# humanoid-path-planner/hpp-fcl

Measured on AMD Instinct MI355X. Metric: narrow-phase queries/s (collision+distance), higher is better.
Workload: dtype f32; 1 GPU; cfg3_convex32_distance_nesterov; request=distance, gather=none

## Files before the change

### hpp-fcl_amd/csrc/hfcl_dev.hpp

```cpp
#pragma once
#include <hip/hip_runtime.h>

#include <cstdint>
#include <cstring>
#include <type_traits>

#include "../../include/hppfcl_amd.h"
#include "hfcl_bvh.hpp"
#include "hfcl_bvh_shape.hpp"
#include "hfcl_pair.hpp"

using namespace hfcl;

#ifndef HFCL_WPE_GJK_W2
#define HFCL_WPE_GJK_W2 2
#endif
#ifndef HFCL_WPE_GJK
#define HFCL_WPE_GJK 3
#endif
#ifndef HFCL_WPE_GJK64
#define HFCL_WPE_GJK64 2
#endif
#ifndef HFCL_WPE_PRIM
#define HFCL_WPE_PRIM 2
#endif
#ifndef HFCL_WPE_EPA32
#define HFCL_WPE_EPA32 2
#endif
#ifndef HFCL_WPE_EPA64
#define HFCL_WPE_EPA64 1
#endif
#ifndef HFCL_WPE_BVH
#define HFCL_WPE_BVH 1
#endif

enum { B_CLOSED = 0, B_PRIM = 1, B_CC = 2, B_PC = 3, B_CP = 4, B_BVH = 5, B_UNSUPPORTED = 6, B_LARGE = 7, B_BVHSHAPE = 8, B_TRI = 9, B_COUNT = 10 };
constexpr int B_CURVED0 = B_COUNT + 4;
constexpr int CTR_SHAPE_TICKET = 2 * B_COUNT + 4, CTR_SHAPE_DEFER = 2 * B_COUNT + 5;
constexpr int CTR_DIST_SUSP = 2 * B_COUNT + 6;
constexpr int CTR_SHAPE_DIST_SUSP = 2 * B_COUNT + 7;
constexpr int CTR_DIST_TICKET = 2 * B_COUNT + 8;
constexpr int CTR_SHAPE_DIST_TICKET = 2 * B_COUNT + 9;
constexpr int CTR_EPA_CC_OVER = 2 * B_COUNT + 10;
constexpr int CTR_SHAPE_FINISH_OVER = 2 * B_COUNT + 11;
constexpr int CTR_SHAPE_DEFER_MARK = 2 * B_COUNT + 13;
constexpr int CTR_DIST_RERUN = 2 * B_COUNT + 14, CTR_SHAPE_DIST_RERUN = 2 * B_COUNT + 15;
constexpr int N_COUNTERS = 2 * B_COUNT + 16;

constexpr int K_CONVEX_LARGE = 21;

__host__ __device__ inline int bucket_of(int k1, int k2, bool distance_mode = false) {
  if (distance_mode && (k1 == K_TRIANGLE || k2 == K_TRIANGLE)) return B_UNSUPPORTED;
  const bool large = (k1 == K_CONVEX_LARGE) || (k2 == K_CONVEX_LARGE);
  if (k1 == K_CONVEX_LARGE) k1 = K_CONVEX;
  if (k2 == K_CONVEX_LARGE) k2 = K_CONVEX;
  if ((k1 == K_BVH) != (k2 == K_BVH)) {
    const int o = (k1 == K_BVH) ? k2 : k1;
    return (kind_is_prim(o) || o == K_CONVEX || kind_is_flat(o)) ? B_BVHSHAPE : B_UNSUPPORTED;
  }
  if ((k1 == K_TRIANGLE || k2 == K_TRIANGLE) && !kind_is_flat(k1) && !kind_is_flat(k2)) {
    const int o = (k1 == K_TRIANGLE) ? k2 : k1;
    return (o == K_TRIANGLE || kind_is_prim(o) || o == K_CONVEX) ? B_TRI : B_UNSUPPORTED;
  }
  const int c = pair_class(k1, k2);
  if (large && c == CLS_CONVEX) return B_LARGE;
  if (c == CLS_CLOSED) return B_CLOSED;
  if (c == CLS_PRIM_GJK) return B_PRIM;
  if (c == CLS_BVH) return B_BVH;
  if (c == CLS_CONVEX) {
    if (k1 == K_CONVEX && k2 == K_CONVEX) return B_CC;
    return (k1 == K_CONVEX) ? B_CP : B_PC;
  }
  return B_UNSUPPORTED;
}

template <typename T>
struct NbrEntry;
template <> struct alignas(16) NbrEntry<float> { float x, y, z; uint32_t id; };
template <> struct alignas(32) NbrEntry<double> { double x, y, z; uint32_t id; uint32_t pad_; };

// ... 657 lines not shown
```

### hpp-fcl_amd/csrc/hfcl_host.hip

```cpp
#include "hfcl_host.hpp"
#include "hfcl_plan.hpp"

static thread_local std::string g_last_error;
void set_error(const std::string& s) { g_last_error = s; }
void hfcl_internal_set_error(const char* msg) { g_last_error = msg ? msg : ""; }

static void free_retired_graphs(hfcl_lib* lib);

static uint32_t total_count(const hfcl_lib* lib, int i) {
  if (lib->last_host) return one_count(lib->acc_counts, i);
  uint32_t c = lib->h_counts ? one_count(lib->h_counts, i) : 0u;
  if (lib->last_split && lib->helper && lib->helper->h_counts) c += one_count(lib->helper->h_counts, i);
  return c;
}

static int ensure_device(int device) {
  int n = 0;
  hipError_t e = hipGetDeviceCount(&n);
  if (e != hipSuccess || n == 0) {
    set_error("no HIP device available (hipGetDeviceCount): the engine has no CPU fallback");
    return HFCL_ERR_NO_DEVICE;
  }
  if (device < 0 || device >= n) {
    set_error("device index out of range");
// ... 149 lines not shown
  }
  lib->h_kinds = kinds;
  std::vector<float> v32(3 * n_vertices + 3);
  for (size_t i = 0; i < 3 * n_vertices; ++i) v32[i] = float(vertices[i]);
  hfcl_lib::Tables& t = lib->own;
  reset_all(t.shapes64, t.shapes32, t.kinds, t.verts64, t.verts32);
  bool ok = true;
  ok = ok && t.shapes64.grow(n_shapes) == hipSuccess;
  ok = ok && t.shapes32.grow(n_shapes) == hipSuccess;
  ok = ok && t.kinds.grow(n_shapes) == hipSuccess;
  ok = ok && t.verts64.grow(3 * n_vertices + 3) == hipSuccess;
  ok = ok && t.verts32.grow(3 * n_vertices + 3) == hipSuccess;
  if (ok) {
    ok = ok && hipMemcpy(t.shapes64, s64.data(), n_shapes * sizeof(DShape<double>), hipMemcpyHostToDevice) == hipSuccess;
    ok = ok && hipMemcpy(t.shapes32, s32.data(), n_shapes * sizeof(DShape<float>), hipMemcpyHostToDevice) == hipSuccess;
    ok = ok && hipMemcpy(t.kinds, kinds.data(), n_shapes, hipMemcpyHostToDevice) == hipSuccess;
    if (n_vertices) {
      ok = ok && hipMemcpy(t.verts64, vertices, 3 * n_vertices * sizeof(double), hipMemcpyHostToDevice) == hipSuccess;
      ok = ok && hipMemcpy(t.verts32, v32.data(), 3 * n_vertices * sizeof(float), hipMemcpyHostToDevice) == hipSuccess;
    }
  }
  share_tables(lib, lib);
  return ok;
}

static const char* const* option_keys() {
  static const char* const keys[] = {
      "closed_staged", "split", "epa_cc_staged", "epa_records_aside", "epa_general_staged", "shape_finish_tiers", "shape_finish_aside",
      "epa_general_staged_min", "epa64_two_streams", "epa_cc_staged_min", "pipe_chunk", "bvh_filter", "bvh_shape_lane", "shape_coop",
      "bvh_cut_ticks", "shape_cut_ticks", "bvh_coop", "bvhd_budget", "bvhd_pool", "shape_dist_pool", "pool_rerun", "bvh_walk_early_coop",
      "bvh_walk_rounds", "bvh_walk_order", "mesh_beside", "mesh_prio", "shape_walk", "shape_walk_sort", "shape_walk_budget", "shape_walk_min", "gjk_beside_max", "epa_direct_max", "bvh_walk_k", "bvh_walk_budget", "shape_dist_leaf_min", "shape_dist_starve", "bvhd_leaf_min", "bvhd_starve",
      "bvhd_part_min", "shape_dist_budget", "bvh_budget0_coop", "shape_budget0", "shape_budget", "shape_leaf_cost", "shape_levels",
      "climb_min", "bvh_budget", "bvh_budget0", "bvh_levels", "cvx_w", "epa_resume_slots", "bvh_task_slots", "bvh_force_wide",
      "pipe_trace", "scene_chunk", "scene_cull_chunk", "scene_pairs_small_max", nullptr};
  return keys;
}
static int parse_list(const char* v, uint32_t* out, int first, int cap, uint32_t lo, uint32_t hi) {
  int k = first;
  for (const char* p = v; *p && k < cap; ++k) {
    const long long x = atoll(p);
    out[k] = uint32_t(std::min<long long>(std::max<long long>(x, lo), hi));
    while (*p && *p != ',') ++p;
    if (*p == ',') ++p;
  }
  return k - first;
}
static int apply_option(hfcl_lib* lib, const std::string& key, const char* v) {
  const long long i = atoll(v);
  const bool on = i != 0;
  auto u32 = [&](long long lo) { return uint32_t(std::min<long long>(std::max(i, lo), 0xFFFFFFFFll)); };
  if (key == "closed_staged") lib->opt.closed_staged = on;
  else if (key == "split") lib->opt.split = i >= 2 ? 2 : (i == 1 ? 1 : 0);
  else if (key == "epa_cc_staged") lib->opt.epa_cc_staged = on;
  else if (key == "epa_records_aside") lib->opt.records_aside = on;
  else if (key == "epa_general_staged") {
    if (on && !HFCL_KEEP_AB_FORMS) return HFCL_ERR_INVALID_ARGUMENT;
    lib->opt.epa_general_staged = on;
  }
  else if (key == "shape_finish_tiers") lib->opt.shape_finish_tiers = on;
  else if (key == "shape_finish_aside") lib->opt.shape_finish_aside = on;
  else if (key == "epa_general_staged_min") lib->opt.epa_general_staged_min = size_t(std::max(0ll, i));
  else if (key == "epa64_two_streams") lib->opt.epa64_two_streams = on;
  else if (key == "epa_cc_staged_min") lib->opt.epa_cc_staged_min = size_t(std::max(0ll, i));
  else if (key == "pipe_chunk") lib->opt.pipe_chunk = strtoull(v, nullptr, 10);
  else if (key == "bvh_filter") {
    if (on && !HFCL_KEEP_AB_FORMS) return HFCL_ERR_INVALID_ARGUMENT;
    lib->opt.bvh_filter = on;
  }
  else if (key == "bvh_shape_lane") lib->opt.bvh_shape_lane = on;
  else if (key == "shape_coop") lib->opt.shape_coop = on;
  else if (key == "bvh_cut_ticks") lib->opt.bvh_cut_ticks = uint32_t(strtoul(v, nullptr, 10));
  else if (key == "shape_cut_ticks") lib->opt.shape_cut_ticks = uint32_t(strtoul(v, nullptr, 10));
  else if (key == "bvh_coop") lib->opt.bvh_coop = on;
  else if (key == "bvhd_budget") lib->opt.bvhd_budget = u32(0);
  else if (key == "bvhd_pool") lib->opt.bvhd_pool = u32(0);
  else if (key == "shape_dist_pool") lib->opt.shape_dist_pool = u32(0);
  else if (key == "pool_rerun") lib->opt.pool_rerun = u32(0);
  else if (key == "bvh_walk_early_coop") lib->opt.walk_early_coop = on;
  else if (key == "bvh_walk_order") lib->opt.walk_order = on;
  else if (key == "mesh_beside") lib->opt.mesh_beside = u32(0);
  else if (key == "shape_walk") lib->opt.shape_walk = on;
  else if (key == "mesh_prio") lib->opt.mesh_prio = on;
  else if (key == "shape_walk_sort") lib->opt.shape_walk_sort = on;
  else if (key == "shape_walk_budget") lib->opt.shape_walk_budget = u32(0);
  else if (key == "shape_walk_min") lib->opt.shape_walk_min = u32(0);
  else if (key == "gjk_beside_max") lib->opt.gjk_beside_max = u32(0);
  else if (key == "epa_direct_max") lib->opt.epa_direct_max = u32(0);
  else if (key == "bvh_walk_rounds") { lib->opt.walk_rounds = uint32_t(std::min<long long>(std::max(0ll, i), WALK_ROUNDS)); lib->opt.walk_auto = false; }
  else if (key == "bvh_walk_k") { parse_list(v, lib->opt.walk_k, 0, WALK_ROUNDS, 1u, uint32_t(WALK_K)); lib->opt.walk_auto = false; }
  else if (key == "bvh_walk_budget") parse_list(v, lib->opt.walk_budget, 1, WALK_ROUNDS, 0u, 0xFFFFFFFFu);
  else if (key == "shape_dist_leaf_min") lib->opt.shape_dist_leaf_min = u32(1);
  else if (key == "shape_dist_starve") lib->opt.shape_dist_starve = u32(1);
  else if (key == "bvhd_leaf_min") lib->opt.bvhd_pool_leaf_min = u32(1);
  else if (key == "bvhd_starve") lib->opt.bvhd_pool_starve = u32(1);
  else if (key == "bvhd_part_min") lib->opt.bvhd_pool_part_min = u32(0);
  else if (key == "shape_dist_budget") lib->opt.shape_dist_budget = u32(0);
  else if (key == "bvh_budget0_coop") lib->opt.bvh_budget0_coop = u32(1);
  else if (key == "shape_budget0") lib->opt.shape_budget0 = lib->opt.shape_budget0_coop = uint32_t(i);
  else if (key == "shape_budget") lib->opt.shape_budget = uint32_t(i);
  else if (key == "shape_leaf_cost") lib->opt.shape_leaf_cost = u32(1);
  else if (key == "shape_levels") lib->opt.shape_levels = uint32_t(std::min<long long>(std::max(1ll, i), BVH_MAX_LEVELS));
  else if (key == "climb_min") lib->opt.climb_min = u32(0);
  else if (key == "bvh_budget") { lib->opt.bvh_budget = lib->opt.bvh_budget0 = u32(0); lib->opt.bvh_auto = false; }
  else if (key == "bvh_budget0") { lib->opt.bvh_budget0 = u32(0); lib->opt.bvh_auto = false; }
  else if (key == "bvh_levels") { lib->opt.bvh_levels = uint32_t(std::min<long long>(BVH_MAX_LEVELS, std::max(1ll, i))); lib->opt.bvh_auto = false; }
  else if (key == "cvx_w") {
    if (i == 0 || i == 2 || i == 4 || i == 8 || i == 16 || i == 32 || i == 64) lib->opt.cvx_w = int(i);
    else return HFCL_ERR_INVALID_ARGUMENT;
  }
  else if (key == "epa_resume_slots") lib->opt.epa_resume_slots = size_t(std::max(0ll, i));
  else if (key == "bvh_task_slots") lib->opt.bvh_task_slots = size_t(std::max(0ll, i));
  else if (key == "bvh_force_wide") lib->opt.bvh_force_wide = on;
  else if (key == "pipe_trace") lib->opt.pipe_trace = on;
  else if (key == "scene_chunk") {
    if (i < 0 || i > 0xFFFFFFF0ll) return HFCL_ERR_INVALID_ARGUMENT;
    lib->opt.scene_chunk = size_t(i);
  }
  else if (key == "scene_cull_chunk") {
    if (i < 0 || i > (1ll << 31)) return HFCL_ERR_INVALID_ARGUMENT;
    lib->opt.scene_cull_chunk = size_t(i);
  }
  else if (key == "scene_pairs_small_max") {
    if (i < 0 || i > (long long)PAIRS_SMALL_MAX) return HFCL_ERR_INVALID_ARGUMENT;
    lib->opt.scene_pairs_small_max = uint32_t(i);
  }
  else return HFCL_ERR_INVALID_ARGUMENT;
  return HFCL_OK;
}

hfcl_lib* hfcl_lib_create(const hfcl_shape* shapes, size_t n_shapes, const double* vertices, size_t n_vertices,
                          int device) {
  if (ensure_device(device) != HFCL_OK) return nullptr;
  if (!validate_shapes("hfcl_lib_create", shapes, n_shapes, vertices, n_vertices)) return nullptr;
  hfcl_lib* lib = new hfcl_lib();
  lib->device = device;
  bool ok = upload_shapes(lib, shapes, n_shapes, vertices, n_vertices);
  ok = ok && lib->d_counts.grow(N_COUNTERS) == hipSuccess;
  ok = ok && lib->h_counts.alloc(N_COUNTERS) == hipSuccess;
  if (ok) memset(lib->h_counts, 0, N_COUNTERS * sizeof(uint32_t));
  if (!ok) {
    set_error("hfcl_lib_create: HIP allocation/copy failed");
    hfcl_lib_destroy(lib);
    return nullptr;
  }
  hipDeviceProp_t prop;
  if (hipGetDeviceProperties(&prop, device) == hipSuccess) lib->n_cus = prop.multiProcessorCount;
  if (lib->d_epa_v0.grow(size_t(lib->n_cus) * 16 * (64 / EPA_WE2) * EPA_MAX_VERTS * sizeof(Quad<double>)) != hipSuccess) {
    set_error("hfcl_lib_create: HIP allocation failed");
    hfcl_lib_destroy(lib);
    return nullptr;
  }
  for (const char* const* k = option_keys(); *k; ++k) {
    std::string name = "HFCL_";
    for (const char* c = *k; *c; ++c) name.push_back(char(toupper(static_cast<unsigned char>(*c))));
    if (const char* v = getenv(name.c_str())) apply_option(lib, *k, v);
  }
  return lib;
}

void hfcl_lib_destroy(hfcl_lib* lib) {
  if (!lib) return;
  hipSetDevice(lib->device);
  hipDeviceSynchronize();
  if (lib->helper) hfcl_lib_destroy(lib->helper);
  delete lib;
}
int hfcl_lib_set_shapes(hfcl_lib* lib, const hfcl_shape* shapes, size_t n_shapes, const double* vertices, size_t n_vertices) {
  if (!lib) {
    set_error("null library");
    return HFCL_ERR_INVALID_ARGUMENT;
// ... 1063 lines not shown
```

### hpp-fcl_amd/csrc/hfcl_host.hpp

```cpp
#pragma once
#include <algorithm>
#include <chrono>
#include <cstdio>
#include <cstdlib>
#include <cstring>
#include <condition_variable>
#include <map>
#include <mutex>
#include <thread>
#include <string>
#include <vector>

#include "hfcl_dev.hpp"
#include "hfcl_launch.hpp"
#include "hfcl_patch.hpp"
#include "hfcl_scene.hpp"
#include "hfcl_cull.hpp"
#include "hfcl_pairs.hpp"
#include "hfcl_own.hpp"

__attribute__((visibility("hidden"))) void set_error(const std::string& s);

#define HIP_TRY(expr)                                                                         \
  do {                                                                                        \
// ... 7 lines not shown
struct KernelTime {
  const char* name;
  Event e0, e1;
  bool used;
};

struct SplitTables {
  DevBuf<BvhTask> tasks;
  DevBuf<void> sums;
  DevBuf<uint32_t> susp, ctr, cut_words;
  DevBuf<double> cut_vals;
  size_t n = 0, cap = 0;
};
struct WalkTables {
  DevBuf<void> recs;
  DevBuf<uint32_t> items;
  DevBuf<void> res;
  DevBuf<uint32_t> lists, ctr, order;
  size_t n = 0;
};

struct hfcl_options {
  uint32_t climb_min = HFCL_CLIMB_MIN;
  uint32_t mesh_beside = 2;
  bool mesh_prio = false;
  uint32_t epa_direct_max = 4096;
  uint32_t gjk_beside_max = 120000;
  bool epa_general_staged = false;
  size_t epa_general_staged_min = 32768;
  bool records_aside = true;
  bool epa64_two_streams = true;
  bool epa_cc_staged = true;
  size_t epa_cc_staged_min = 32768;
  bool shape_finish_tiers = true;
  bool shape_finish_aside = true;
  bool bvh_shape_lane = true;
  uint32_t shape_budget0 = 128, shape_budget = 96, shape_leaf_cost = 32, shape_levels = BVH_MAX_LEVELS;
  bool shape_coop = true;
  uint32_t bvh_cut_ticks = 0, shape_cut_ticks = 350000;
  uint32_t shape_budget0_coop = 16;
  bool bvh_coop = true;
  uint32_t bvh_budget0_coop = 0;
  uint32_t bvhd_budget = 64;
  uint32_t bvhd_pool = 1;
  uint32_t bvhd_pool_leaf_min = 24, bvhd_pool_starve = 32, bvhd_pool_part_min = 48;
  uint32_t pool_rerun = 1;
  uint32_t shape_dist_pool = 1;
  uint32_t shape_dist_leaf_min = 48, shape_dist_starve = 16;
  uint32_t shape_dist_budget = 64;
  size_t pipe_chunk = 0;
  int split = 0;
  size_t scene_cull_chunk = 0;
  uint32_t scene_pairs_small_max = 32;
  size_t scene_chunk = 0;
  int cvx_w = 0;
  bool closed_staged = true;
  bool bvh_filter = false;
  bool walk_order = true;
  bool shape_walk_sort = true;
  bool shape_walk = true;
  uint32_t shape_walk_budget = 256;
  uint32_t shape_walk_min = 65536;
  size_t epa_resume_slots = 0, bvh_task_slots = 0;
  bool bvh_force_wide = false, pipe_trace = false;
  bool walk_early_coop = true;
  bool walk_auto = true;
// ... 204 lines not shown
```

### hpp-fcl_amd/csrc/hfcl_host_batch.hip

```cpp
#include "hfcl_host.hpp"

static int ensure_workspace(hfcl_lib* lib, size_t n, bool need_epa) {
  if (n > lib->ws_capacity) {
    lib->ws_capacity = 0;
    const size_t cap = n + n / 8 + 1024;
    HIP_TRY(lib->d_lists.grow(size_t(B_COUNT) * cap));
    lib->ws_capacity = cap;
  }
  if (need_epa && lib->ws_capacity > lib->epa_capacity) {
    reset_all(lib->d_epa_queue, lib->d_epa_queue2, lib->d_epa_resume, lib->d_epa_cc_over);
    lib->resume_cap = 0;
    lib->epa_capacity = 0;
    const size_t cap = lib->ws_capacity;
    HIP_TRY(lib->d_epa_queue.grow(cap * sizeof(EpaItem<double>)));
    HIP_TRY(lib->d_epa_queue2.grow(cap * sizeof(EpaItem<double>)));
    size_t rcap = std::min(cap, std::max<size_t>(65536, cap / 8));
    if (lib->opt.epa_resume_slots) rcap = std::max<size_t>(1, std::min<size_t>(cap, lib->opt.epa_resume_slots));
    HIP_TRY(lib->d_epa_resume.grow(rcap * std::max(epa_resume_stride<double>, epa_resume_stride<float>)));
    HIP_TRY(lib->d_epa_cc_over.grow(rcap));
    lib->resume_cap = rcap;
    lib->epa_capacity = cap;
  }
  return HFCL_OK;
}
// ... 512 lines not shown
  if (gen_staged) {
    HIP_TRY(lib->d_epa_ready_g.grow(lib->ws_capacity * sizeof(EpaReadyG<T>)));
    wk.epa_ready_g = lib->d_epa_ready_g;
  }
  if constexpr (F32) {
    if (cc_staged) {
      Timed t(b, "k_epa_prepare", st);
      launch_epa_prepare(b.blocks_for(n / 4 + 1, 256), st, wk, b.lv, b.io, b.q);
    }
  }
  if (gen_staged) {
    Timed t(b, "k_epa_prepare_general", st);
    launch_epa_prepare_general<T>(b.blocks_for(n / 4 + 1, 256), st, wk, b.lv, b.io, b.q, F32);
  }
  if (direct) {
    Timed t(b, "k_epa<full>", st);
    launch_epa_requeue<T>(st, wk);
    launch_epa_full<T>(int(std::min<size_t>(b.blocks_for(n / 2 + 1, 64 / epa_we2<T>), size_t(lib->n_cus) * 16)), st, wk, b.lv, b.io, b.q);
    return HFCL_OK;
  }
  const int epa_batches = int(std::min<size_t>((n + 64 / EPA_WE - 1) / (64 / EPA_WE), size_t(1) << 22));
  {
    Timed t(b, "k_epa<fast>", st);
    hipStream_t st2 = nullptr;
    if constexpr (!F32) {
      if (o.epa64_two_streams && lib->has_curved && general_q) {
        if (int rc = ensure_aux(lib)) return rc;
        st2 = lib->aux;
        HIP_TRY(hipEventRecord(lib->ev_aux0, st));
        HIP_TRY(hipStreamWaitEvent(st2, lib->ev_aux0, 0));
      }
    }
    if constexpr (F32)
      if (cc_staged) launch_epa_loop(epa_batches, st, wk, b.lv, b.q, lib->n_cus);
    if (gen_staged) launch_epa_loop_general<T>(epa_batches, st, st2, wk, b.lv, b.q, lib->n_cus, lib->has_curved);
    if ((F32 && b.may(B_CC) && !cc_staged) || (general_q && !gen_staged))
      launch_epa_fast<T>(epa_batches, st, wk, b.lv, b.io, b.q, b.may(B_CC) && !cc_staged, general_q && !gen_staged, lib->n_cus, lib->has_curved, st2);
    if (st2) {
      HIP_TRY(hipEventRecord(lib->ev_aux1, st2));
      HIP_TRY(hipStreamWaitEvent(st, lib->ev_aux1, 0));
    }
  }
  if (!(cc_staged || gen_staged)) {
    Timed t(b, "k_epa<full>", st);
    launch_epa_full<T>(b.blocks_for(n / 16 + 1, 64 / epa_we2<T>), st, wk, b.lv, b.io, b.q);
    return HFCL_OK;
  }
  const bool aside = o.records_aside;
  if (aside) {
    if (int rc = ensure_aux(lib)) return rc;
    HIP_TRY(hipEventRecord(lib->ev_aux0, st));
    HIP_TRY(hipStreamWaitEvent(lib->aux, lib->ev_aux0, 0));
  }
  hipStream_t const rs = aside ? lib->aux.get() : st;
  {
    Timed t(b, "k_epa_records", rs);
    if constexpr (F32)
      if (cc_staged) launch_epa_records(b.blocks_for(n / 4 + 1, 256), rs, wk, b.lv, b.io, b.q);
    if (gen_staged) launch_epa_records_general<T>(b.blocks_for(n / 4 + 1, 256), rs, wk, b.lv, b.io, b.q, F32);
  }
  hipStream_t const fs = cc_staged ? rs : st;
  {
    Timed t(b, "k_epa<full>", fs);
    launch_epa_full<T>(b.blocks_for(n / 16 + 1, 64 / epa_we2<T>), fs, wk, b.lv, b.io, b.q);
  }
  if (aside) HIP_TRY(hipEventRecord(lib->ev_aux1, rs));
  if constexpr (F32) {
// ... 6 lines not shown
  return HFCL_OK;
}

template <typename T>
static int finish_batch(Batch<T>& b, hipStream_t st) {
  hfcl_lib* lib = b.lib;
  {
    Timed t(b, "k_unsupported", st);
    if (b.may(B_UNSUPPORTED)) launch_unsupported<T>(b.blocks_for(b.n, 256 * 64), st, b.wk, b.io, int(B_UNSUPPORTED));
    if (lib->h_meshes.empty()) {
      if (b.may(B_BVHSHAPE)) launch_unsupported<T>(b.blocks_for(b.n, 256 * 64), st, b.wk, b.io, int(B_BVHSHAPE));
      if (b.may(B_BVH)) launch_unsupported<T>(b.blocks_for(b.n, 256 * 64), st, b.wk, b.io, int(B_BVH));
    }
  }
  HIP_TRY(hipMemcpyAsync(lib->counts_dst ? lib->counts_dst : lib->h_counts.get(), lib->d_counts, N_COUNTERS * sizeof(uint32_t), hipMemcpyDeviceToHost, st));
  lib->ran_batch = lib->counts_dst == nullptr;
  HIP_TRY(hipGetLastError());
  return HFCL_OK;
}

template <typename T>
static int run_batch_one(hfcl_lib* lib, const uint32_t* d_s1, const uint32_t* d_s2, IO<T> io, size_t n, QParams<T> q, hipStream_t st) {
  if (n == 0) return HFCL_OK;
  if (n > 0xFFFFFFF0ull) {
    set_error("batch too large (max 2^32-16 pairs per call)");
    return HFCL_ERR_LIMIT;
  }
  HIP_TRY(hipSetDevice(lib->device));
  Batch<T> b{lib, Work(), LibView<T>(), io, q, n};
  int rc = ensure_workspace(lib, n, b.any_gjk() && q.compute_penetration);
  if (rc) return rc;
  make_views(b, d_s1, d_s2);
  for (auto& t : lib->timers) t.used = false;
  HIP_TRY(hipMemsetAsync(lib->d_counts, 0, N_COUNTERS * sizeof(uint32_t), st));
  {
    Timed t(b, "k_classify", st);
    launch_classify(b.blocks_for(n, CLS_BLOCK * 8), st, b.wk, lib->d_kinds, uint32_t(lib->n_shapes), q.mode != 1);
  }
  bool mesh_join_pending = false;
  if (meshes_run_beside(b)) {
    HIP_TRY(hipEventRecord(lib->ev_mesh_fork, st));
    HIP_TRY(hipStreamWaitEvent(lib->mesh_st, lib->ev_mesh_fork, 0));
    rc = launch_meshes(b, lib->mesh_st.get(), true);
    if (rc) return rc;
    HIP_TRY(hipEventRecord(lib->ev_mesh_join, lib->mesh_st));
    rc = launch_solids(b, st);
    if (rc) return rc;
    if (lib->opt.mesh_beside < 2) HIP_TRY(hipStreamWaitEvent(st, lib->ev_mesh_join, 0));
    else mesh_join_pending = true;
  } else {
    rc = launch_solids(b, st);
    if (rc) return rc;
    rc = launch_meshes(b, st, false);
    if (rc) return rc;
  }
  if (q.compute_penetration && b.any_gjk()) {
    rc = launch_epa(b, st);
    if (rc) return rc;
  }
  if (mesh_join_pending) HIP_TRY(hipStreamWaitEvent(st, lib->ev_mesh_join, 0));
  return finish_batch(b, st);
}

void share_tables(hfcl_lib* h, const hfcl_lib* lib) {
  const hfcl_lib::Tables& t = lib->own;
  h->n_shapes = lib->n_shapes;
  h->d_shapes64 = t.shapes64;
  h->d_shapes32 = t.shapes32;
  h->d_verts64 = t.verts64;
  h->d_verts32 = t.verts32;
  h->d_kinds = t.kinds;
  h->possible_buckets = lib->possible_buckets;
  h->has_curved = lib->has_curved;
  h->has_flats = lib->has_flats;
  h->d_graph_base = t.graph.base;
  h->d_graph_off = t.graph.off;
  h->d_graph_ent32 = t.graph.ent32;
  h->d_graph_ent64 = t.graph.ent64;
}
static hfcl_lib* make_helper(hfcl_lib* lib) {
  hfcl_lib* h = new hfcl_lib;
  h->device = lib->device;
  share_tables(h, lib);
  h->n_cus = lib->n_cus;
  bool ok = h->d_counts.grow(N_COUNTERS) == hipSuccess;
  ok = ok && h->h_counts.alloc(N_COUNTERS) == hipSuccess;
  ok = ok && h->d_epa_v0.grow(size_t(h->n_cus) * 16 * (64 / EPA_WE2) * EPA_MAX_VERTS * sizeof(Quad<double>)) == hipSuccess;
  if (!ok) {
    hfcl_lib_destroy(h);
    return nullptr;
  }
  memset(h->h_counts, 0, N_COUNTERS * sizeof(uint32_t));
  return h;
}

template <typename T>
static IO<T> io_at(const IO<T>& io, size_t lo) {
  const size_t w = std::is_same<T, double>::value ? 12 : 7;
  return IO<T>{io.tf1 + w * lo, io.tf2 + w * lo, io.out + lo, io.gin ? io.gin + lo : nullptr, io.gout ? io.gout + lo : nullptr};
}

bool batch_splits(const hfcl_lib* lib, size_t n) {
  constexpr size_t MIN_SPLIT = 1u << 17;
  int parts = lib->opt.split;
  if (parts == 0) {
    int kinds = 0;
    for (int b : {int(B_PRIM), int(B_CC), int(B_PC), int(B_CP), int(B_LARGE)}) kinds += (lib->possible_buckets >> b) & 1u;
    parts = kinds >= 3 ? 2 : 1;
  }
  return parts >= 2 && n >= MIN_SPLIT && lib->h_meshes.empty();
}
int ensure_helper(hfcl_lib* lib) {
  if (lib->helper) return HFCL_OK;
  HIP_TRY(hipSetDevice(lib->device));
  hfcl_lib* h = make_helper(lib);
  Stream side;
  Event fork, join;
  if (!h || side.create() != hipSuccess || fork.create() != hipSuccess || join.create() != hipSuccess) {
// ... 43 lines not shown
```

### hpp-fcl_amd/csrc/hfcl_k_epa.hip

```cpp
#include <algorithm>

#include "hfcl_dev.hpp"
#include "hfcl_launch.hpp"

#ifndef HFCL_UNIT_PRECISION
#define HFCL_UNIT_PRECISION 0
#endif
#define HFCL_UNIT_F32 (HFCL_UNIT_PRECISION != 64)
#define HFCL_UNIT_F64 (HFCL_UNIT_PRECISION != 32)

template <typename T, int WE, bool LARGE>
struct EpaSupport {
  DShape<T> a, b;
  HullRegs<T, WE> h0, h1;
  const T* va;
  const T* vb;
  HullGraph<T> ga, gb;
  mutable int hint0, hint1;
  MDiff<T> md;
  int lig;
  __device__ __forceinline__ V3<T> hull(const DShape<T>& s, const HullRegs<T, WE>& h, const T* v, const HullGraph<T>& g, const V3<T>& d, int& hint) const {
    if (LARGE && s.num_points > uint32_t(HULL_MAX)) return large_hull_support<T, WE>(v, s.num_points, g, d, lig, hint);
    return h.support(d, lig);
  }
// ... 292 lines not shown
          res.status = EPA_FALLBACK;
          res.iterations = 0;
          PairOut<T> o;
          epa_finish(res, ip->gjk_iters, load_pose(io.tf1, pair), T(0), T(0), o);
          write_out<T>(io, q, pair, o);
          write_guess<T>(io, pair, o.cached_guess, 0, 0);
        }
      }
    }
    if (live) {
      ready[i] = rb;
    } else {
      ready[i].packed = 0u;
      ready[i].state = EPA_READY_NONE;
    }
  }
}

#ifndef HFCL_EPA_LOOP_REFILL_MIN
#define HFCL_EPA_LOOP_REFILL_MIN 2
#endif
#ifndef HFCL_EPA_LOOP_ROUNDS
#define HFCL_EPA_LOOP_ROUNDS 1
#endif
#ifndef HFCL_EPA_CC_RESUME
#define HFCL_EPA_CC_RESUME 1
#endif
template <typename T>
__device__ __forceinline__ EpaSaved<T, EPA_FAST_CAP>* cc_resume_slot(const Work& wk, uint32_t slot) {
  return resume_slot<T, EPA_FAST_CAP>(wk, wk.cc_resume_base + slot);
}
template <typename T, int WE, int CAP>
__global__ void __launch_bounds__(64) __attribute__((amdgpu_waves_per_eu(HFCL_WPE_EPA32_CC, 8)))
k_epa_loop(Work wk, LibView<T> lib, QParams<T> q) {
  constexpr int G = 64 / WE;
  static_assert(WE >= 8, "a group's lanes copy the eight records of a block");
  typedef LaneGroup<WE> Grp;
  __shared__ EpaScratch<T, CAP, V0_TAG> scratch[G];
  const uint32_t cnt = wk.counts[B_COUNT + 3];
  const int lane = threadIdx.x & 63, grp = lane / WE, lig = lane & (WE - 1);
  EpaReady<T>* const ready = reinterpret_cast<EpaReady<T>*>(wk.epa_ready);
  const EpaItem<T>* const queue = reinterpret_cast<const EpaItem<T>*>(wk.epa_queue);
  enum { IDLE = 0, LIVE = 1, DONE = 2, HANDOVER = 3 };
  int state = IDLE;
  uint32_t it = 0;
  uint32_t next = blockIdx.x;
  EpaSupportCC<T, WE> sup;
  sup.lig = lig;
  Epa<T, Grp, CAP, V0_TAG> epa;
  EpaLoop<T> L;
  while (true) {
    const uint64_t live = __ballot(state == LIVE);
    const int n_live = __popcll(live) / WE;
    const bool more = next < cnt;
    if (n_live == 0 || (more && G - n_live >= HFCL_EPA_LOOP_REFILL_MIN)) {
      if (state != LIVE) {
        if (state != IDLE) {
          EpaReady<T>* rb = ready + it;
          if (state == DONE) {
            EpaLoopOut<T> o;
            epa.loop_out(L, o);
            if (lig == 0) {
              *reinterpret_cast<EpaLoopOut<T>*>(rb->md) = o;
              rb->state = EPA_READY_DONE;
            }
          } else {
            uint32_t slot = 0xFFFFFFFFu;
            if (HFCL_EPA_CC_RESUME && epa.resumable) {
              if (lig == 0) slot = atomicAdd(&wk.counts[CTR_EPA_CC_OVER], 1u);
              slot = __shfl(slot, 0, WE);
            }
            if (slot < wk.cc_resume_cap) {
              epa_save_block<T, Grp, CAP, V0_TAG, NoTags, true>(&scratch[grp], cc_resume_slot<T>(wk, slot));
              if (lig == 0) wk.epa_cc_over[slot] = it;
            } else {
              if (lig == 0) {
                const EpaItem<T>* ip = queue + (wk.n - 1u - rb->seed);
                const uint32_t s2 = atomicAdd(&wk.counts[B_COUNT + 1], 1u);
                reinterpret_cast<EpaItem<T>*>(wk.epa_queue2)[s2] = *ip;
              }
            }
            if (lig == 0) rb->state = EPA_READY_HANDED_OVER;
          }
          Grp::sync();
          state = IDLE;
        }
        const uint64_t lower = live | ~((uint64_t(1) << (grp * WE)) - 1);
        const uint32_t rank = uint32_t(__popcll(~lower)) / WE;
        it = next + rank * gridDim.x;
        if (it < cnt) {
          const EpaReady<T>* rb = ready + it;
          const uint32_t packed = rb->packed;
          if ((packed & 63u) != 0u) {
          sup.h0.load(lib.verts + 3 * size_t(rb->voff_a), packed & 63u, lig);
          sup.h1.load(lib.verts + 3 * size_t(rb->voff_b), (packed >> 6) & 63u, lig);
          sup.md.oR1.r0 = mk<T>(rb->md[0], rb->md[1], rb->md[2]);
          sup.md.oR1.r1 = mk<T>(rb->md[3], rb->md[4], rb->md[5]);
          sup.md.oR1.r2 = mk<T>(rb->md[6], rb->md[7], rb->md[8]);
          sup.md.ot1 = mk<T>(rb->md[9], rb->md[10], rb->md[11]);
          sup.md.identity = (packed >> 18) & 1u;
          epa.reset(&scratch[grp], q.epa_max_iterations, q.epa_tolerance);
          epa.loop_enter(L, epa.install(rb, packed), 0, 0);
          state = LIVE;
          }
        }
      }
      next += uint32_t(G - n_live) * gridDim.x;
      if (n_live == 0 && !more) {
        if (__ballot(state == LIVE) == 0) break;
      }
      continue;
    }
    if (state == LIVE) {
      const int r = epa.step(L, sup);
      if (r != 0) state = r == 1 ? DONE : HANDOVER;
    }
  }
}

template <typename T, int WE>
__global__ void __launch_bounds__(64) k_epa_resume_cc(Work wk, LibView<T> lib, IO<T> io, QParams<T> q) {
  constexpr int G = 64 / WE, CAP = EPA_MAX_ITER;
  typedef LaneGroup<WE> Grp;
  __shared__ EpaScratch<T, CAP, V0_TAG> scratch[G];
  const uint32_t cnt = min(wk.counts[CTR_EPA_CC_OVER], wk.cc_resume_cap);
  const int lane = threadIdx.x & 63, grp = lane / WE, lig = lane & (WE - 1);
  const EpaReady<T>* const ready = reinterpret_cast<const EpaReady<T>*>(wk.epa_ready);
  const EpaItem<T>* const queue = reinterpret_cast<const EpaItem<T>*>(wk.epa_queue);
  for (uint32_t it = blockIdx.x * G + grp; it < cnt; it += gridDim.x * G) {
    const uint32_t idx = wk.epa_cc_over[it];
    if (idx == 0xFFFFFFFFu) continue;
    const EpaReady<T>* rb = ready + idx;
    const uint32_t packed = rb->packed, pair = rb->pair;
    EpaSupportCC<T, WE> sup;
    sup.lig = lig;
    const T* va = lib.verts + 3 * size_t(rb->voff_a);
    sup.h0.load(va, packed & 63u, lig);
    sup.h1.load(lib.verts + 3 * size_t(rb->voff_b), (packed >> 6) & 63u, lig);
    sup.md.oR1.r0 = mk<T>(rb->md[0], rb->md[1], rb->md[2]);
    sup.md.oR1.r1 = mk<T>(rb->md[3], rb->md[4], rb->md[5]);
// ... 243 lines not shown
}
template <typename T>
void launch_epa_fast(int grid, hipStream_t st, const Work& wk, const LibView<T>& lv, const IO<T>& io, const QParams<T>& q, bool cc_queue, bool general_queue, int n_cus, bool curved_class, hipStream_t st2) {
  if constexpr (sizeof(T) == 4) {
    static const int per_cu_cc = resident_blocks_per_cu(k_epa_stream<T, EPA_WE, EPA_FAST_CAP, true>);
    static const int per_cu_gen = resident_blocks_per_cu(k_epa_stream<T, EPA_WE, EPA_FAST_CAP, false>);
    if (cc_queue)
      hipLaunchKernelGGL((k_epa_stream<T, EPA_WE, EPA_FAST_CAP, true>), dim3(std::min(grid, n_cus * per_cu_cc * HFCL_EPA_GRID_ROUNDS)), dim3(64), 0, st, wk, lv, io, q);
    if (general_queue)
      hipLaunchKernelGGL((k_epa_stream<T, EPA_WE, EPA_FAST_CAP, false>), dim3(std::min(grid, n_cus * per_cu_gen * HFCL_EPA_GRID_ROUNDS)), dim3(64), 0, st, wk, lv, io, q);
  } else {
#ifdef HFCL_EPA64_STREAM_CURVED
    static const int per_cu = resident_blocks_per_cu(k_epa_stream<T, HFCL_EPA64_CURVED_WE, epa_fast_cap<T>, false, true>);
    hipLaunchKernelGGL((k_epa_stream<T, HFCL_EPA64_CURVED_WE, epa_fast_cap<T>, false, true>), dim3(std::min(grid * (HFCL_EPA64_CURVED_WE / EPA_WE), n_cus * per_cu * HFCL_EPA_GRID_ROUNDS)), dim3(64), 0, st, wk, lv, io, q);
    hipLaunchKernelGGL((k_epa<T, EPA_WE, epa_small_cap<T>, 1, 1>), dim3(std::min(grid, n_cus * 32)), dim3(64), 0, st, wk, lv, io, q);
#else
    if (curved_class)
      hipLaunchKernelGGL((k_epa<T, HFCL_EPA64_CURVED_WE, epa_fast_cap<T>, 1, 2>), dim3(std::min(grid * (HFCL_EPA64_CURVED_WE / EPA_WE), n_cus * 16)), dim3(64), 0, st, wk, lv, io, q);
    hipLaunchKernelGGL((k_epa<T, EPA_WE, epa_small_cap<T>, 1, 1>), dim3(std::min(grid, n_cus * 32)), dim3(64), 0, (curved_class && st2) ? st2 : st, wk, lv, io, q);
#endif
  }
}
#if HFCL_UNIT_F32
template void launch_epa_fast<float>(int, hipStream_t, const Work&, const LibView<float>&, const IO<float>&, const QParams<float>&, bool, bool, int, bool, hipStream_t);
#endif
#if HFCL_UNIT_F64
template void launch_epa_fast<double>(int, hipStream_t, const Work&, const LibView<double>&, const IO<double>&, const QParams<double>&, bool, bool, int, bool, hipStream_t);
#endif

#if HFCL_UNIT_F32
void launch_epa_prepare(int grid, hipStream_t st, const Work& wk, const LibView<float>& lv, const IO<float>& io, const QParams<float>& q) {
  hipLaunchKernelGGL((k_epa_prepare<float>), dim3(grid), dim3(256), 0, st, wk, lv, io, q);
}
void launch_epa_loop(int grid, hipStream_t st, const Work& wk, const LibView<float>& lv, const QParams<float>& q, int n_cus) {
  static const int per_cu = resident_blocks_per_cu(k_epa_loop<float, EPA_WE, EPA_FAST_CAP>);
  hipLaunchKernelGGL((k_epa_loop<float, EPA_WE, EPA_FAST_CAP>), dim3(std::min(grid, n_cus * per_cu * HFCL_EPA_LOOP_ROUNDS)), dim3(64), 0, st, wk, lv, q);
}
void launch_epa_resume_cc(int grid, hipStream_t st, const Work& wk, const LibView<float>& lv, const IO<float>& io, const QParams<float>& q) {
  hipLaunchKernelGGL((k_epa_resume_cc<float, HFCL_EPA_CC_RESUME_WE>), dim3(grid), dim3(64), 0, st, wk, lv, io, q);
}
void launch_epa_records(int grid, hipStream_t st, const Work& wk, const LibView<float>& lv, const IO<float>& io, const QParams<float>& q) {
  hipLaunchKernelGGL((k_epa_records<float>), dim3(grid), dim3(256), 0, st, wk, lv, io, q);
}

#endif

#if !HFCL_KEEP_AB_FORMS
template <typename T> void launch_epa_prepare_general(int, hipStream_t, const Work&, const LibView<T>&, const IO<T>&, const QParams<T>&, bool) {}
template <typename T> void launch_epa_records_general(int, hipStream_t, const Work&, const LibView<T>&, const IO<T>&, const QParams<T>&, bool) {}
template <typename T> void launch_epa_loop_general(int, hipStream_t, hipStream_t, const Work&, const LibView<T>&, const QParams<T>&, int, bool) {}
#else
template <typename T>
void launch_epa_prepare_general(int grid, hipStream_t st, const Work& wk, const LibView<T>& lv, const IO<T>& io, const QParams<T>& q, bool skip_top) {
  hipLaunchKernelGGL((k_epa_prepare_general<T>), dim3(grid), dim3(256), 0, st, wk, lv, io, q, skip_top ? 1 : 0);
}
template <typename T>
void launch_epa_records_general(int grid, hipStream_t st, const Work& wk, const LibView<T>& lv, const IO<T>& io, const QParams<T>& q, bool skip_top) {
  hipLaunchKernelGGL((k_epa_records_general<T>), dim3(grid), dim3(256), 0, st, wk, lv, io, q, skip_top ? 1 : 0);
}
#ifndef HFCL_EPA_LOOPG_ROUNDS
#define HFCL_EPA_LOOPG_ROUNDS 1
#endif
template <typename T>
void launch_epa_loop_general(int grid, hipStream_t st, hipStream_t st2, const Work& wk, const LibView<T>& lv, const QParams<T>& q, int n_cus, bool curved_class) {
  if constexpr (sizeof(T) == 4) {
    static const int per_cu = resident_blocks_per_cu(k_epa_loop_general<T, EPA_WE, EPA_FAST_CAP, false>);
    hipLaunchKernelGGL((k_epa_loop_general<T, EPA_WE, EPA_FAST_CAP, false>), dim3(std::min(grid, n_cus * per_cu * HFCL_EPA_LOOPG_ROUNDS)), dim3(64), 0, st, wk, lv, q);
  } else {
    static const int per_cu_c = resident_blocks_per_cu(k_epa_loop_general<T, HFCL_EPA64_CURVED_WE, epa_fast_cap<T>, true>);
// ... 49 lines not shown
```

### hpp-fcl_amd/csrc/hfcl_launch.hpp

```cpp
#pragma once
#include "hfcl_dev.hpp"

void launch_classify(int grid, hipStream_t st, const Work& wk, const uint8_t* kinds, uint32_t n_shapes, bool distance_mode);
template <typename T> void launch_unsupported(int grid, hipStream_t st, const Work& wk, const IO<T>& io, int bucket);
template <typename T> void launch_closed(int grid, hipStream_t st, const Work& wk, const LibView<T>& lv, const IO<T>& io, const QParams<T>& q, bool staged);
template <typename T> void launch_gjk_prim(int grid, hipStream_t st, const Work& wk, const LibView<T>& lv, const IO<T>& io, const QParams<T>& q, bool bvg);
template <typename T> constexpr int gjk_cvx_threads(int w, int m) { return (sizeof(T) == 4 && w == 2 && m == 0) ? 64 : 256; }
template <typename T> void launch_gjk_cvx(int m, int w, bool bvg, int grid, hipStream_t st, const Work& wk, const LibView<T>& lv, const IO<T>& io, const QParams<T>& q);
template <typename T> void launch_gjk_large(int grid, hipStream_t st, const Work& wk, const LibView<T>& lv, const IO<T>& io, const QParams<T>& q, bool bvg);
void launch_expand_poses(hipStream_t st, const double* qt, double* tf, uint32_t n);
void launch_fill_skipped(hipStream_t st, hfcl_result* out, uint32_t n);
void launch_fill_skipped(hipStream_t st, hfcl_result_f32* out, uint32_t n);
void launch_compact_records(hipStream_t st, const hfcl_result* in, hfcl_result_compact* out, uint32_t n);
void launch_compact_records(hipStream_t st, const hfcl_result_f32* in, hfcl_result_compact_f32* out, uint32_t n);

template <typename T> void launch_epa_fast(int grid, hipStream_t st, const Work& wk, const LibView<T>& lv, const IO<T>& io, const QParams<T>& q, bool cc_queue, bool general_queue, int n_cus, bool curved_class = true, hipStream_t st2 = nullptr);
void launch_epa_prepare(int grid, hipStream_t st, const Work& wk, const LibView<float>& lv, const IO<float>& io, const QParams<float>& q);
void launch_epa_loop(int grid, hipStream_t st, const Work& wk, const LibView<float>& lv, const QParams<float>& q, int n_cus);
void launch_epa_resume_cc(int grid, hipStream_t st, const Work& wk, const LibView<float>& lv, const IO<float>& io, const QParams<float>& q);
void launch_epa_records(int grid, hipStream_t st, const Work& wk, const LibView<float>& lv, const IO<float>& io, const QParams<float>& q);
template <typename T> void launch_epa_prepare_general(int grid, hipStream_t st, const Work& wk, const LibView<T>& lv, const IO<T>& io, const QParams<T>& q, bool skip_top);
template <typename T> void launch_epa_loop_general(int grid, hipStream_t st, hipStream_t st2, const Work& wk, const LibView<T>& lv, const QParams<T>& q, int n_cus, bool curved_class);
template <typename T> void launch_epa_records_general(int grid, hipStream_t st, const Work& wk, const LibView<T>& lv, const IO<T>& io, const QParams<T>& q, bool skip_top);
template <typename T> void launch_epa_requeue(hipStream_t st, const Work& wk);
template <typename T> void launch_epa_full(int grid, hipStream_t st, const Work& wk, const LibView<T>& lv, const IO<T>& io, const QParams<T>& q);

struct AsideStream {
  hipStream_t stream;
  hipEvent_t fork, join;
};
template <typename T> void launch_bvh_collide(int grid, hipStream_t st, const Work& wk, const LibView<T>& lv, const BvhView<T>& bv, const IO<T>& io, const QParams<T>& q, const BvhParams& bp, T break_distance2, BvhSplit split, BvhSpill spill, const AsideStream* aside = nullptr);
template <typename T> void launch_bvh_distance(int grid, hipStream_t st, const Work& wk, const LibView<T>& lv, const BvhView<T>& bv, const IO<T>& io, const QParams<T>& q, BvhSpill spill);
template <typename T> void launch_bvh_shape(int grid, hipStream_t st, const Work& wk, const LibView<T>& lv, const BvhView<T>& bv, const IO<T>& io, const QParams<T>& q, const BvhParams& bp, T break_distance2);
template <typename T> void launch_bvh_shape_distance_fast(int grid, int grid_finish, hipStream_t st, const Work& wk, const LibView<T>& lv, const BvhView<T>& bv, const IO<T>& io, const QParams<T>& q, BvhSpill spill);
template <typename T> void launch_bvh_shape_fast(int grid, int grid_finish, int coop_grid, hipStream_t st, const Work& wk, const LibView<T>& lv, const BvhView<T>& bv, const IO<T>& io, const QParams<T>& q, const BvhParams& bp, T break_distance2, BvhSplit split, BvhSpill spill, const AsideStream* aside = nullptr);
template <typename T> void launch_bvh_shape_distance(int grid, hipStream_t st, const Work& wk, const LibView<T>& lv, const BvhView<T>& bv, const IO<T>& io, const QParams<T>& q);
template <typename T> void launch_triangle(int grid, hipStream_t st, const Work& wk, const LibView<T>& lv, const IO<T>& io, const QParams<T>& q);

struct PatchArgs {
  const uint32_t* s1;
  const uint32_t* s2;
  const double* tf1;
  const double* tf2;
  const hfcl_result* rec;
  const hfcl_guess* guess;
  uint32_t n, n_shapes;
  const DShape<double>* shapes;
  const double* verts;
  const uint32_t* graph_base;
  const uint32_t* graph_off;
  const uint32_t* graph_ent;
// ... 138 lines not shown
```

Measured before the change: 614.4 million queries/s.

## Add atomic work-stealing pool for the tail of the staged EPA loop

The staged f32 EPA loop now processes most items with the existing static grid stride, then hands a configurable share of the tail to a pool of sixteen ticketed ranges. Blocks claim ranges through atomic counters padded to separate cache lines. This targets the load imbalance at the end of the loop, where some blocks finish early while others still hold long EPA runs. The cost is extra atomics, a larger counter region to clear on each batch, and two new tuning options.

```diff
diff --git a/hpp-fcl_amd/csrc/hfcl_dev.hpp b/hpp-fcl_amd/csrc/hfcl_dev.hpp
--- a/hpp-fcl_amd/csrc/hfcl_dev.hpp
+++ b/hpp-fcl_amd/csrc/hfcl_dev.hpp
@@ -8,6 +8,7 @@
 #include "../../include/hppfcl_amd.h"
 #include "hfcl_bvh.hpp"
 #include "hfcl_bvh_shape.hpp"
+#include "hfcl_epa_pool.hpp"
 #include "hfcl_pair.hpp"
 
 using namespace hfcl;
@@ -46,6 +47,8 @@
 constexpr int CTR_SHAPE_DEFER_MARK = 2 * B_COUNT + 13;
 constexpr int CTR_DIST_RERUN = 2 * B_COUNT + 14, CTR_SHAPE_DIST_RERUN = 2 * B_COUNT + 15;
 constexpr int N_COUNTERS = 2 * B_COUNT + 16;
+constexpr int EPA_POOL_CTR0 = (N_COUNTERS + EPA_POOL_STRIDE_WORDS - 1) / EPA_POOL_STRIDE_WORDS * EPA_POOL_STRIDE_WORDS;
+constexpr int N_COUNTER_WORDS = EPA_POOL_CTR0 + EPA_POOL_K * EPA_POOL_STRIDE_WORDS;
 
 constexpr int K_CONVEX_LARGE = 21;
 
diff --git a/hpp-fcl_amd/csrc/hfcl_epa_pool.hpp b/hpp-fcl_amd/csrc/hfcl_epa_pool.hpp
--- /dev/null
+++ b/hpp-fcl_amd/csrc/hfcl_epa_pool.hpp
@@ -0,0 +1,47 @@
+#pragma once
+#include <cstdint>
+
+#include "hfcl_math.hpp"
+
+namespace hfcl {
+
+constexpr int EPA_POOL_K = 16;
+constexpr int EPA_POOL_STRIDE_WORDS = 32;
+
+struct EpaPoolPlan {
+  uint32_t S;
+  uint32_t len;
+};
+
+HFCL_HD EpaPoolPlan epa_pool_plan(uint32_t cnt, uint32_t grid, uint32_t groups, uint32_t share_pct, uint32_t min_refills, uint32_t k) {
+  EpaPoolPlan p{cnt, 0u};
+  if (share_pct == 0u || grid == 0u || k == 0u) return p;
+  if (uint64_t(cnt) < uint64_t(grid) * groups * min_refills) return p;
+  const uint32_t pool = uint32_t(uint64_t(cnt) * share_pct / 100u);
+  p.S = (cnt - pool) / grid * grid;
+  p.len = uint32_t((uint64_t(cnt - p.S) + k - 1u) / k);
+  return p;
+}
+HFCL_HD uint32_t epa_pool_range_base(const EpaPoolPlan& p, uint32_t j) { return p.S + j * p.len; }
+HFCL_HD uint32_t epa_pool_range_len(const EpaPoolPlan& p, uint32_t cnt, uint32_t j) {
+  const uint64_t lo = uint64_t(p.S) + uint64_t(j) * p.len;
+  if (lo >= cnt) return 0u;
+  const uint64_t left = cnt - lo;
+  return left < p.len ? uint32_t(left) : p.len;
+}
+HFCL_HD uint32_t epa_pool_take(uint32_t t, uint32_t want, uint32_t len) {
+  if (t >= len) return 0u;
+  const uint32_t left = len - t;
+  return want < left ? want : left;
+}
+HFCL_HD bool epa_pool_drained(uint32_t t, uint32_t want, uint32_t len) { return uint64_t(t) + want >= len; }
+HFCL_HD uint32_t epa_pool_pick(uint32_t dry, uint32_t at, uint32_t k) {
+  for (uint32_t s = 0; s < k; ++s) {
+    const uint32_t j = at + s < k ? at + s : at + s - k;
+    if (!((dry >> j) & 1u)) return j;
+  }
+  return k;
+}
+HFCL_HD uint32_t epa_pool_full_mask(uint32_t k) { return k >= 32u ? 0xFFFFFFFFu : (1u << k) - 1u; }
+
+}
diff --git a/hpp-fcl_amd/csrc/hfcl_host.hip b/hpp-fcl_amd/csrc/hfcl_host.hip
--- a/hpp-fcl_amd/csrc/hfcl_host.hip
+++ b/hpp-fcl_amd/csrc/hfcl_host.hip
@@ -205,7 +205,7 @@
       "bvh_walk_rounds", "bvh_walk_order", "mesh_beside", "mesh_prio", "shape_walk", "shape_walk_sort", "shape_walk_budget", "shape_walk_min", "gjk_beside_max", "epa_direct_max", "bvh_walk_k", "bvh_walk_budget", "shape_dist_leaf_min", "shape_dist_starve", "bvhd_leaf_min", "bvhd_starve",
       "bvhd_part_min", "shape_dist_budget", "bvh_budget0_coop", "shape_budget0", "shape_budget", "shape_leaf_cost", "shape_levels",
       "climb_min", "bvh_budget", "bvh_budget0", "bvh_levels", "cvx_w", "epa_resume_slots", "bvh_task_slots", "bvh_force_wide",
-      "pipe_trace", "scene_chunk", "scene_cull_chunk", "scene_pairs_small_max", nullptr};
+      "pipe_trace", "scene_chunk", "scene_cull_chunk", "scene_pairs_small_max", "epa_pool_share", "epa_pool_min_refills", nullptr};
   return keys;
 }
 static int parse_list(const char* v, uint32_t* out, int first, int cap, uint32_t lo, uint32_t hi) {
@@ -259,6 +259,11 @@
   else if (key == "shape_walk_min") lib->opt.shape_walk_min = u32(0);
   else if (key == "gjk_beside_max") lib->opt.gjk_beside_max = u32(0);
   else if (key == "epa_direct_max") lib->opt.epa_direct_max = u32(0);
+  else if (key == "epa_pool_share") {
+    if (i < 0 || i > 50) return HFCL_ERR_INVALID_ARGUMENT;
+    lib->opt.epa_pool_share = uint32_t(i);
+  }
+  else if (key == "epa_pool_min_refills") lib->opt.epa_pool_min_refills = u32(0);
   else if (key == "bvh_walk_rounds") { lib->opt.walk_rounds = uint32_t(std::min<long long>(std::max(0ll, i), WALK_ROUNDS)); lib->opt.walk_auto = false; }
   else if (key == "bvh_walk_k") { parse_list(v, lib->opt.walk_k, 0, WALK_ROUNDS, 1u, uint32_t(WALK_K)); lib->opt.walk_auto = false; }
   else if (key == "bvh_walk_budget") parse_list(v, lib->opt.walk_budget, 1, WALK_ROUNDS, 0u, 0xFFFFFFFFu);
@@ -308,7 +313,7 @@
   hfcl_lib* lib = new hfcl_lib();
   lib->device = device;
   bool ok = upload_shapes(lib, shapes, n_shapes, vertices, n_vertices);
-  ok = ok && lib->d_counts.grow(N_COUNTERS) == hipSuccess;
+  ok = ok && lib->d_counts.grow(N_COUNTER_WORDS) == hipSuccess;
   ok = ok && lib->h_counts.alloc(N_COUNTERS) == hipSuccess;
   if (ok) memset(lib->h_counts, 0, N_COUNTERS * sizeof(uint32_t));
   if (!ok) {
diff --git a/hpp-fcl_amd/csrc/hfcl_host.hpp b/hpp-fcl_amd/csrc/hfcl_host.hpp
--- a/hpp-fcl_amd/csrc/hfcl_host.hpp
+++ b/hpp-fcl_amd/csrc/hfcl_host.hpp
@@ -63,6 +63,7 @@
   bool epa64_two_streams = true;
   bool epa_cc_staged = true;
   size_t epa_cc_staged_min = 32768;
+  uint32_t epa_pool_share = 20, epa_pool_min_refills = 2;
   bool shape_finish_tiers = true;
   bool shape_finish_aside = true;
   bool bvh_shape_lane = true;
diff --git a/hpp-fcl_amd/csrc/hfcl_host_batch.hip b/hpp-fcl_amd/csrc/hfcl_host_batch.hip
--- a/hpp-fcl_amd/csrc/hfcl_host_batch.hip
+++ b/hpp-fcl_amd/csrc/hfcl_host_batch.hip
@@ -568,7 +568,7 @@
       }
     }
     if constexpr (F32)
-      if (cc_staged) launch_epa_loop(epa_batches, st, wk, b.lv, b.q, lib->n_cus);
+      if (cc_staged) launch_epa_loop(epa_batches, st, wk, b.lv, b.q, lib->n_cus, o.epa_pool_share, o.epa_pool_min_refills);
     if (gen_staged) launch_epa_loop_general<T>(epa_batches, st, st2, wk, b.lv, b.q, lib->n_cus, lib->has_curved);
     if ((F32 && b.may(B_CC) && !cc_staged) || (general_q && !gen_staged))
       launch_epa_fast<T>(epa_batches, st, wk, b.lv, b.io, b.q, b.may(B_CC) && !cc_staged, general_q && !gen_staged, lib->n_cus, lib->has_curved, st2);
@@ -641,7 +641,7 @@
   if (rc) return rc;
   make_views(b, d_s1, d_s2);
   for (auto& t : lib->timers) t.used = false;
-  HIP_TRY(hipMemsetAsync(lib->d_counts, 0, N_COUNTERS * sizeof(uint32_t), st));
+  HIP_TRY(hipMemsetAsync(lib->d_counts, 0, N_COUNTER_WORDS * sizeof(uint32_t), st));
   {
     Timed t(b, "k_classify", st);
     launch_classify(b.blocks_for(n, CLS_BLOCK * 8), st, b.wk, lib->d_kinds, uint32_t(lib->n_shapes), q.mode != 1);
@@ -692,7 +692,7 @@
   h->device = lib->device;
   share_tables(h, lib);
   h->n_cus = lib->n_cus;
-  bool ok = h->d_counts.grow(N_COUNTERS) == hipSuccess;
+  bool ok = h->d_counts.grow(N_COUNTER_WORDS) == hipSuccess;
   ok = ok && h->h_counts.alloc(N_COUNTERS) == hipSuccess;
   ok = ok && h->d_epa_v0.grow(size_t(h->n_cus) * 16 * (64 / EPA_WE2) * EPA_MAX_VERTS * sizeof(Quad<double>)) == hipSuccess;
   if (!ok) {
diff --git a/hpp-fcl_amd/csrc/hfcl_k_epa.hip b/hpp-fcl_amd/csrc/hfcl_k_epa.hip
--- a/hpp-fcl_amd/csrc/hfcl_k_epa.hip
+++ b/hpp-fcl_amd/csrc/hfcl_k_epa.hip
@@ -348,12 +348,18 @@
 }
 template <typename T, int WE, int CAP>
 __global__ void __launch_bounds__(64) __attribute__((amdgpu_waves_per_eu(HFCL_WPE_EPA32_CC, 8)))
-k_epa_loop(Work wk, LibView<T> lib, QParams<T> q) {
+k_epa_loop(Work wk, LibView<T> lib, QParams<T> q, uint32_t pool_share, uint32_t pool_min_refills) {
   constexpr int G = 64 / WE;
   static_assert(WE >= 8, "a group's lanes copy the eight records of a block");
   typedef LaneGroup<WE> Grp;
   __shared__ EpaScratch<T, CAP, V0_TAG> scratch[G];
   const uint32_t cnt = wk.counts[B_COUNT + 3];
+  constexpr uint32_t K = EPA_POOL_K, POOL_FULL = (1u << K) - 1u;
+  const EpaPoolPlan pool = epa_pool_plan(cnt, gridDim.x, G, pool_share, pool_min_refills, K);
+  const uint32_t S = pool.S;
+  uint32_t* const tickets = wk.counts + EPA_POOL_CTR0;
+  uint32_t dry = pool.len ? 0u : POOL_FULL;
+  uint32_t at = blockIdx.x % K;
   const int lane = threadIdx.x & 63, grp = lane / WE, lig = lane & (WE - 1);
   EpaReady<T>* const ready = reinterpret_cast<EpaReady<T>*>(wk.epa_ready);
   const EpaItem<T>* const queue = reinterpret_cast<const EpaItem<T>*>(wk.epa_queue);
@@ -368,8 +374,26 @@
   while (true) {
     const uint64_t live = __ballot(state == LIVE);
     const int n_live = __popcll(live) / WE;
-    const bool more = next < cnt;
+    const bool strided = next < S;
+    const bool more = strided || dry != POOL_FULL;
     if (n_live == 0 || (more && G - n_live >= HFCL_EPA_LOOP_REFILL_MIN)) {
+      uint32_t drawn = 0, n_drawn = 0;
+      if (!strided && dry != POOL_FULL) {
+        const uint32_t want = uint32_t(G - n_live);
+        while (dry != POOL_FULL) {
+          at = epa_pool_pick(dry, at, K);
+          uint32_t t = 0u;
+          if (lane == 0) t = __hip_atomic_fetch_add(tickets + at * EPA_POOL_STRIDE_WORDS, want, __ATOMIC_RELAXED, __HIP_MEMORY_SCOPE_AGENT);
+          t = __builtin_amdgcn_readfirstlane(t);
+          const uint32_t len_at = epa_pool_range_len(pool, cnt, at);
+          n_drawn = epa_pool_take(t, want, len_at);
+          if (epa_pool_drained(t, want, len_at)) dry |= 1u << at;
+          if (n_drawn) {
+            drawn = epa_pool_range_base(pool, at) + t;
+            break;
+          }
+        }
+      }
       if (state != LIVE) {
         if (state != IDLE) {
           EpaReady<T>* rb = ready + it;
@@ -403,8 +427,8 @@
         }
         const uint64_t lower = live | ~((uint64_t(1) << (grp * WE)) - 1);
         const uint32_t rank = uint32_t(__popcll(~lower)) / WE;
-        it = next + rank * gridDim.x;
-        if (it < cnt) {
+        it = strided ? next + rank * gridDim.x : drawn + rank;
+        if (strided ? it < S : rank < n_drawn) {
           const EpaReady<T>* rb = ready + it;
           const uint32_t packed = rb->packed;
           if ((packed & 63u) != 0u) {
@@ -421,7 +445,7 @@
           }
         }
       }
-      next += uint32_t(G - n_live) * gridDim.x;
+      if (strided) next += uint32_t(G - n_live) * gridDim.x;
       if (n_live == 0 && !more) {
         if (__ballot(state == LIVE) == 0) break;
       }
@@ -731,9 +755,9 @@
 void launch_epa_prepare(int grid, hipStream_t st, const Work& wk, const LibView<float>& lv, const IO<float>& io, const QParams<float>& q) {
   hipLaunchKernelGGL((k_epa_prepare<float>), dim3(grid), dim3(256), 0, st, wk, lv, io, q);
 }
-void launch_epa_loop(int grid, hipStream_t st, const Work& wk, const LibView<float>& lv, const QParams<float>& q, int n_cus) {
+void launch_epa_loop(int grid, hipStream_t st, const Work& wk, const LibView<float>& lv, const QParams<float>& q, int n_cus, uint32_t pool_share, uint32_t pool_min_refills) {
   static const int per_cu = resident_blocks_per_cu(k_epa_loop<float, EPA_WE, EPA_FAST_CAP>);
-  hipLaunchKernelGGL((k_epa_loop<float, EPA_WE, EPA_FAST_CAP>), dim3(std::min(grid, n_cus * per_cu * HFCL_EPA_LOOP_ROUNDS)), dim3(64), 0, st, wk, lv, q);
+  hipLaunchKernelGGL((k_epa_loop<float, EPA_WE, EPA_FAST_CAP>), dim3(std::min(grid, n_cus * per_cu * HFCL_EPA_LOOP_ROUNDS)), dim3(64), 0, st, wk, lv, q, pool_share, pool_min_refills);
 }
 void launch_epa_resume_cc(int grid, hipStream_t st, const Work& wk, const LibView<float>& lv, const IO<float>& io, const QParams<float>& q) {
   hipLaunchKernelGGL((k_epa_resume_cc<float, HFCL_EPA_CC_RESUME_WE>), dim3(grid), dim3(64), 0, st, wk, lv, io, q);
diff --git a/hpp-fcl_amd/csrc/hfcl_launch.hpp b/hpp-fcl_amd/csrc/hfcl_launch.hpp
--- a/hpp-fcl_amd/csrc/hfcl_launch.hpp
+++ b/hpp-fcl_amd/csrc/hfcl_launch.hpp
@@ -16,7 +16,7 @@
 
 template <typename T> void launch_epa_fast(int grid, hipStream_t st, const Work& wk, const LibView<T>& lv, const IO<T>& io, const QParams<T>& q, bool cc_queue, bool general_queue, int n_cus, bool curved_class = true, hipStream_t st2 = nullptr);
 void launch_epa_prepare(int grid, hipStream_t st, const Work& wk, const LibView<float>& lv, const IO<float>& io, const QParams<float>& q);
-void launch_epa_loop(int grid, hipStream_t st, const Work& wk, const LibView<float>& lv, const QParams<float>& q, int n_cus);
+void launch_epa_loop(int grid, hipStream_t st, const Work& wk, const LibView<float>& lv, const QParams<float>& q, int n_cus, uint32_t pool_share, uint32_t pool_min_refills);
 void launch_epa_resume_cc(int grid, hipStream_t st, const Work& wk, const LibView<float>& lv, const IO<float>& io, const QParams<float>& q);
 void launch_epa_records(int grid, hipStream_t st, const Work& wk, const LibView<float>& lv, const IO<float>& io, const QParams<float>& q);
 template <typename T> void launch_epa_prepare_general(int grid, hipStream_t st, const Work& wk, const LibView<T>& lv, const IO<T>& io, const QParams<T>& q, bool skip_top);
```

Measured after the change: 645.7 million queries/s (median of 6 runs). +5.1%, better.
